# Qualcomm-AI-research/transformer-quantization

Measured on AMD Instinct MI355X. Metric: M elems/sec fake-quant fwd (BERT-base act tensor); achieved HBM GB/s vs peak, higher is better.
Workload: dtype f32; 1 GPU; BERT-base W8A8 per-tensor asym 8-bit activation fake-quant, running-minmax calibrated, fixed-range fwd, hidden [1024,512,768] bf16 per GPU (BASELINE configs[1]); storage_dtype=bf16, parallelism=dp1 (independent shards, no data-path collective)

## Files before the change

transformer-quantization_amd/csrc/tq_linear_i8.hip:

```cpp
#include <algorithm>
#include <type_traits>

#include "tq_device.h"
#include "tq_host.h"

namespace tq {

typedef int v4i __attribute__((ext_vector_type(4)));

enum { ACT_NONE = 0, ACT_RELU = 1, ACT_GELU = 2, ACT_TANH = 3 };

__device__ __forceinline__ float apply_act(float v, int act) {
  switch (act) {
    case ACT_RELU: return v > 0.0f ? v : 0.0f;
    case ACT_GELU: return 0.5f * v * (1.0f + erff(v * 0.70710678118654752440f));
    case ACT_TANH: return tanhf(v);
    default: return v;
  }
}

struct LinArgs {
  const int8_t* x;
  const int8_t* w;
  const int32_t* w_rowsum;
// ... 426 lines not shown
    if (GROUPED && p.split_out && grp == 2) w.t2sel = p.q_t2c;
    w.q1 = load_qraw(p.q_t1, 0, p.x_delta);
    w.q2 = load_qraw(w.t2sel, 0, p.x_delta);
  }
  w.st[0] = w.st[1] = w.st[2] = w.st[3] = 0.0f;
  if (!WITH_TAIL && p.stair != nullptr) {
#pragma unroll
    for (int i = 0; i < 4; ++i) w.st[i] = p.stair[i];
  }
  return w;
}

template <bool WITH_TAIL>
__device__ __forceinline__ void epilogue_arrived(EpiRaw& w) {
  w.dx = pinned_uniform(w.dx);
  w.zx = pinned_uniform(w.zx);
  qraw_arrived(w.qo);
  if (WITH_TAIL) { qraw_arrived(w.q1); qraw_arrived(w.q2); }
  else {
#pragma unroll
    for (int i = 0; i < 4; ++i) w.st[i] = pinned_uniform(w.st[i]);
  }
}

template <bool WITH_TAIL, bool SEL = false>
__device__ __forceinline__ EpiCtx epilogue_finish(const LinArgs& p, const EpiRaw& w) {
  EpiCtx c;
  c.sx = w.dx < p.x_eps ? p.x_eps : w.dx;
  const int zx = (int)clamp_nanprop(rintf(w.zx), 0.0f, grid_top(p.x_n_bits));
  c.shift = 128 - zx;
  c.qo = QP{1.f, 0.f, 0.f, 0.f};
  if (p.has_q) c.qo = qp_from_raw<SEL>(w.qsel, w.qo);
  c.qf = make_qf(c.qo);
  c.fast = p.act != ACT_TANH && (!p.has_q || c.qf.ok) && p.fast_epi != 0;
  c.stair = false;
  c.st_inv_w = c.st_c0 = c.st_nbm1 = 0.0f;
  if (!WITH_TAIL && p.stair != nullptr && p.has_q && c.fast) {
    c.st_inv_w = w.st[0]; c.st_c0 = w.st[1]; c.st_nbm1 = w.st[2];
    c.stair = w.st[3] == 1.0f && c.st_nbm1 == (float)(p.stair_bins - 1);
  }
  c.qf1 = c.qf2 = c.qf;
  if (WITH_TAIL) {
    c.qf1 = make_qf(p.on_t1 ? qp_from_raw<SEL>(p.q_t1, w.q1) : QP{1.f, 0.f, 0.f, 1.f});
    c.qf2 = make_qf(p.on_t2 ? qp_from_raw<SEL>(w.t2sel, w.q2) : QP{1.f, 0.f, 0.f, 1.f});
    c.fast = c.fast && p.act == ACT_NONE && c.qf1.ok && c.qf2.ok;
  }
  return c;
}

template <bool WITH_TAIL>
__device__ __forceinline__ EpiCtx epilogue_prepare(const LinArgs& p, uint32_t n0) {
  EpiRaw w = epilogue_fetch<WITH_TAIL>(p, n0);
  epilogue_arrived<WITH_TAIL>(w);
  return epilogue_finish<WITH_TAIL>(p, w);
}

template <int NI, int MI, int YDT, bool STAGED, bool WITH_TAIL, bool FLUSH = true, bool FPRE = false>
__device__ __forceinline__ void linear_epilogue(const LinArgs& p, v4i (&acc)[NI][MI], uint32_t n0, uint32_t m0, int r16,
                                                int kg, const EpiCtx& c, int8_t* stage = nullptr, const float* cst = nullptr,
                                                int cs = 2 * NI * 16, const f32x4 (*res_pre)[MI] = nullptr,
                                                const u32x2* stair_lds = nullptr) {
  static_assert(!(FPRE && WITH_TAIL), "class-ordered input grids: no fused tail");
  if (!c.fast) return linear_epilogue_generic<NI, MI, YDT, FPRE>(p, acc, n0, m0, r16, kg, c.qo, c.shift, c.sx, res_pre, FLUSH ? nullptr : stage);
  if (WITH_TAIL) {
#define TQ_EPI_T(Q, T) linear_epilogue_fast<NI, MI, YDT, ACT_NONE, Q, STAGED, T, FLUSH>(p, acc, n0, m0, r16, kg, c.qf, c.shift, c.sx, stage, cst, c.qf1, c.qf2, cs, res_pre)
    if (p.tail == 2) { if (p.has_q) TQ_EPI_T(true, 2); else TQ_EPI_T(false, 2); }
    else             { if (p.has_q) TQ_EPI_T(true, 1); else TQ_EPI_T(false, 1); }
#undef TQ_EPI_T
    return;
  }
#define TQ_EPI(A, Q) linear_epilogue_fast<NI, MI, YDT, A, Q, STAGED, 0, true, FPRE>(p, acc, n0, m0, r16, kg, c.qf, c.shift, c.sx, stage, cst, QF{}, QF{}, cs)
  if (STAGED && c.stair && stair_lds != nullptr) {
    linear_epilogue_stair<NI, MI, YDT, FPRE>(p, acc, n0, m0, r16, kg, c.qf, stage, cst, cs, StairRef{stair_lds, c.st_inv_w, c.st_c0, c.st_nbm1});
    return;
  }
  if (p.has_q) {
    if (p.act == ACT_GELU)      TQ_EPI(ACT_GELU, true);
    else if (p.act == ACT_RELU) TQ_EPI(ACT_RELU, true);
    else                        TQ_EPI(ACT_NONE, true);
  } else {
    if (p.act == ACT_GELU)      TQ_EPI(ACT_GELU, false);
    else if (p.act == ACT_RELU) TQ_EPI(ACT_RELU, false);
    else                        TQ_EPI(ACT_NONE, false);
  }
#undef TQ_EPI
}

template <int TN, int TM, int YDT, bool WITH_TAIL>
__global__ __launch_bounds__(kBlock) void linear_i8_k(LinArgs p) {
  constexpr int NI = TN / 16, MI = TM / 16;
  const int lane = threadIdx.x & 63;
  const uint32_t tiles_m = p.M / TM;
  const uint32_t tile = blockIdx.x * (kBlock / kWave) + (threadIdx.x >> 6);
  if (tile >= tiles_m * (p.N / TN)) return;
  const uint32_t n0 = (tile / tiles_m) * TN, m0 = (tile % tiles_m) * TM;

  const int r16 = lane & 15, kg = lane >> 4;
  const int8_t* wp = p.w + (size_t)(n0 + r16) * p.K + kg * 16;
  const int8_t* xp = p.x + (size_t)(m0 + r16) * p.K + kg * 16;

  v4i acc[NI][MI];
#pragma unroll
  for (int i = 0; i < NI; ++i)
#pragma unroll
    for (int j = 0; j < MI; ++j) acc[i][j] = v4i{0, 0, 0, 0};

  v4i fw[NI], fx[MI];
#pragma unroll
  for (int i = 0; i < NI; ++i) fw[i] = *reinterpret_cast<const v4i*>(wp + (size_t)i * 16 * p.K);
#pragma unroll
  for (int j = 0; j < MI; ++j) fx[j] = *reinterpret_cast<const v4i*>(xp + (size_t)j * 16 * p.K);

  for (uint32_t k = 64; k <= p.K; k += 64) {
    v4i nw[NI], nx[MI];
    const bool more = k < p.K;
    if (more) {
#pragma unroll
      for (int i = 0; i < NI; ++i) nw[i] = *reinterpret_cast<const v4i*>(wp + (size_t)i * 16 * p.K + k);
#pragma unroll
      for (int j = 0; j < MI; ++j) nx[j] = *reinterpret_cast<const v4i*>(xp + (size_t)j * 16 * p.K + k);
    }
#pragma unroll
    for (int i = 0; i < NI; ++i)
#pragma unroll
      for (int j = 0; j < MI; ++j)
        acc[i][j] = __builtin_amdgcn_mfma_i32_16x16x64_i8(fw[i], fx[j], acc[i][j], 0, 0, 0);
    if (more) {
#pragma unroll
      for (int i = 0; i < NI; ++i) fw[i] = nw[i];
#pragma unroll
      for (int j = 0; j < MI; ++j) fx[j] = nx[j];
    }
  }
  linear_epilogue<NI, MI, YDT, false, WITH_TAIL>(p, acc, n0, m0, r16, kg, epilogue_prepare<WITH_TAIL>(p, n0));
}

__device__ __forceinline__ void lds_dma_wait_all() { asm volatile("s_waitcnt vmcnt(0)" ::: "memory"); }

#define TQ_GLDS16(gp, lp)                                                                         \
  __builtin_amdgcn_global_load_lds((const __attribute__((address_space(1))) void*)(gp),           \
                                   (__attribute__((address_space(3))) void*)(lp), 16, 0, 0)

template <int N>
__device__ __forceinline__ void lds_dma_wait_but() {
  asm volatile("s_waitcnt vmcnt(%0)" ::"n"(N) : "memory");
}

struct ClsArgs {
  uint32_t n;
  uint32_t end_slab[TQ_CLS_MAX];
  uint32_t rep[TQ_CLS_MAX];
};

template <int WT, int YDT, bool WITH_TAIL, int NS, bool CLS, bool X16 = false>
__device__ __forceinline__ void linear_i8_lds_body(const LinArgs& p, const ClsArgs* ct, const int8_t* x_lo = nullptr) {
  static_assert(NS == 2 || NS == 8, "double buffer or the 8-stage ring");
  static_assert(!CLS || (NS == 2 && !WITH_TAIL), "class-ordered input grids: double buffer, no tail");
  static_assert(!X16 || (NS == 2 && !WITH_TAIL && !CLS), "16-bit input grids: double buffer, no tail, per-tensor");
  constexpr int BT = 2 * WT, NI = WT / 16, MI = WT / 16;
  constexpr int LPW = WT / 16;
  constexpr int OPB = BT * 128, STB = (X16 ? 3 : 2) * OPB;
  extern __shared__ __attribute__((aligned(1024))) int8_t lds_i8[];
  prefetch_kernarg<sizeof(LinArgs)>();
  const int tid = threadIdx.x, lane = tid & 63, wave = __builtin_amdgcn_readfirstlane(tid >> 6);
  const uint32_t tiles_m = p.M / BT;
  const int wn = (wave >> 1) * WT, wm = (wave & 1) * WT;
  const int r16 = lane & 15, kg = lane >> 4;
  const int swz = (r16 >> 1) & 7;
  const int off[2] = {r16 * 128 + ((kg ^ swz) << 4), r16 * 128 + (((4 + kg) ^ swz) << 4)};
  float* cst = reinterpret_cast<float*>(lds_i8 + NS * STB);
  float* csx = reinterpret_cast<float*>(lds_i8 + NS * STB + 5 * BT * 4);
  int* csh = reinterpret_cast<int*>(csx + TQ_CLS_MAX);
  int* crs = csh + TQ_CLS_MAX;
  const uint32_t cls_bytes = CLS ? 2 * TQ_CLS_MAX * 4 + ct->n * BT * 4 : 0;
  u32x2* stab = reinterpret_cast<u32x2*>(lds_i8 + NS * STB + 5 * BT * 4 + cls_bytes);
  const uint32_t nk = p.K / 128;

  {
    const uint32_t tile = blockIdx.x;
    const uint32_t n0 = (tile / tiles_m) * BT, m0 = (tile % tiles_m) * BT;
    const int8_t* wsrc[LPW];
    const int8_t* xsrc[LPW];
    const int8_t* x2src[X16 ? LPW : 1];
#pragma unroll
    for (int q = 0; q < LPW; ++q) {
      const int row = wave * (WT / 2) + q * 8 + (lane >> 3);
      const int chunk = (lane & 7) ^ ((row >> 1) & 7);
      wsrc[q] = p.w + (size_t)(n0 + row) * p.K + chunk * 16;
      xsrc[q] = p.x + (size_t)(m0 + row) * p.K + chunk * 16;
      if (X16) x2src[X16 ? q : 0] = x_lo + (size_t)(m0 + row) * p.K + chunk * 16;
    }
    auto issue = [&](int stage, uint32_t k) {
#ifdef TQ_I8_DBG_BUILD
      if (p.dbg & 2) return;
#endif
      int8_t* bw = lds_i8 + stage * STB + wave * (WT / 2) * 128;
#pragma unroll
      for (int q = 0; q < LPW; ++q) {
        TQ_GLDS16(wsrc[q] + k, bw + q * 1024);
        TQ_GLDS16(xsrc[q] + k, bw + OPB + q * 1024);
        if (X16) TQ_GLDS16(x2src[X16 ? q : 0] + k, bw + 2 * OPB + q * 1024);
      }
    };

    v4i acc[NI][MI];
    f32x4 facc[CLS ? NI : 1][CLS ? MI : 1];
    v4i acc2[X16 ? NI : 1][X16 ? MI : 1];
#pragma unroll
    for (int i = 0; i < NI; ++i)
#pragma unroll
      for (int j = 0; j < MI; ++j) acc[i][j] = v4i{0, 0, 0, 0};
    if (X16) {
#pragma unroll
      for (int i = 0; i < (X16 ? NI : 1); ++i)
#pragma unroll
        for (int j = 0; j < (X16 ? MI : 1); ++j) acc2[i][j] = v4i{0, 0, 0, 0};
    }
    if (CLS) {
#pragma unroll
      for (int i = 0; i < (CLS ? NI : 1); ++i)
#pragma unroll
        for (int j = 0; j < (CLS ? MI : 1); ++j) facc[i][j] = f32x4{-0.0f, -0.0f, -0.0f, -0.0f};
    }
    uint32_t cls = 0, cls_end = CLS ? ct->end_slab[0] : 0;

    EpiRaw eraw = epilogue_fetch<WITH_TAIL>(p, n0 + wn);
    const uint32_t ncol = n0 + (tid & (BT - 1));
    const float ld_dw = p.w_delta[p.w_n_params == 1 ? 0 : ncol], ld_b = p.bias ? p.bias[ncol] : 0.0f;
    const int ld_rs = CLS ? 0 : p.w_rowsum[ncol];
    float ld_nw = 0.0f, ld_nb = 0.0f;
    if (WITH_TAIL) { ld_nw = p.nn_w[ncol]; ld_nb = p.nn_b[ncol]; }
    if (CLS) {
      if (tid < BT)
        for (uint32_t c = 0; c < ct->n; ++c) crs[c * BT + tid] = p.w_rowsum[(size_t)c * p.N + ncol];
      if (tid == 0)
        for (uint32_t c = 0; c < ct->n; ++c) {
          const float dxc = p.x_delta[ct->rep[c]], zfc = p.x_zero_float[ct->rep[c]];
          csx[c] = dxc < p.x_eps ? p.x_eps : dxc;
          csh[c] = 128 - (int)clamp_nanprop(rintf(zfc), 0.0f, grid_top(p.x_n_bits));
        }
    }
#pragma unroll
    for (int s = 0; s < (NS == 2 ? 2 : NS - 2); ++s)
      if ((uint32_t)s < nk) issue(s, s * 128);
    epilogue_arrived<WITH_TAIL>(eraw);
    const EpiCtx ectx = epilogue_finish<WITH_TAIL, WT == 64>(p, eraw);
    if (tid < BT) {
      cst[tid] = CLS ? (ld_dw < p.w_eps ? p.w_eps : ld_dw) : ectx.sx * (ld_dw < p.w_eps ? p.w_eps : ld_dw);
      cst[BT + tid] = ld_b;
      reinterpret_cast<int*>(cst)[2 * BT + tid] = X16 ? ld_rs : ld_rs * ectx.shift;
      if (WITH_TAIL) { cst[3 * BT + tid] = ld_nw; cst[4 * BT + tid] = ld_nb; }
    }
    if (!WITH_TAIL && ectx.stair) {
      const u32x2* gtab = reinterpret_cast<const u32x2*>(p.stair + 4);
      for (uint32_t i = tid; i < p.stair_bins; i += kBlock) stab[i] = gtab[i];
    }
    for (uint32_t kb = 0; kb < nk; ++kb) {
      if (NS == 2) {
        lds_dma_wait_all();
        __syncthreads();
        if (kb > 0 && kb + 1 < nk) issue((kb + 1) & 1, (kb + 1) * 128);
      } else if ((kb & 1) == 0) {
        constexpr int IPS = 2 * LPW;
        const uint32_t rest = nk - 2 - kb;
        if (rest >= (uint32_t)(NS - 4)) lds_dma_wait_but<(NS - 4) * IPS>();
        else if (rest == 2) lds_dma_wait_but<2 * IPS>();
        else lds_dma_wait_but<0>();
        asm volatile("s_barrier" ::: "memory");
        if (kb + NS - 2 < nk) {
          issue((kb + NS - 2) % NS, (kb + NS - 2) * 128);
          issue((kb + NS - 1) % NS, (kb + NS - 1) * 128);
        }
      }
      const int8_t* bw = lds_i8 + (kb % NS) * STB + wn * 128;
      const int8_t* bx = lds_i8 + (kb % NS) * STB + OPB + wm * 128;
      v4i fw[2][NI], fx[2][MI], fx2[2][X16 ? MI : 1];
      auto load_frags = [&](int s2) {
#pragma unroll
        for (int i = 0; i < NI; ++i) fw[s2][i] = *reinterpret_cast<const v4i*>(bw + i * 2048 + off[s2]);
#pragma unroll
        for (int j = 0; j < MI; ++j) fx[s2][j] = *reinterpret_cast<const v4i*>(bx + j * 2048 + off[s2]);
        if (X16) {
#pragma unroll
          for (int j = 0; j < (X16 ? MI : 1); ++j) fx2[s2][j] = *reinterpret_cast<const v4i*>(bx + OPB + j * 2048 + off[s2]);
        }
      };
      load_frags(0);
#pragma unroll
      for (int s = 0; s < 2; ++s) {
        if (s == 0) load_frags(1);
        __builtin_amdgcn_sched_barrier(0);
#ifdef TQ_I8_DBG_BUILD
        if (p.dbg & 4) {
#pragma unroll
          for (int i = 0; i < NI; ++i) acc[i][0] = acc[i][0] + fw[s][i] + fx[s][i % MI];
          continue;
        }
#endif
#pragma unroll
        for (int i = 0; i < NI; ++i)
#pragma unroll
          for (int j = 0; j < MI; ++j)
            acc[i][j] = __builtin_amdgcn_mfma_i32_16x16x64_i8(fw[s][i], fx[s][j], acc[i][j], 0, 0, 0);
        if (X16) {
#pragma unroll
          for (int i = 0; i < (X16 ? NI : 1); ++i)
#pragma unroll
            for (int j = 0; j < (X16 ? MI : 1); ++j)
              acc2[i][j] = __builtin_amdgcn_mfma_i32_16x16x64_i8(fw[s][i], fx2[s][j], acc2[i][j], 0, 0, 0);
        }
      }
      if (CLS && kb + 1 == cls_end) {
        const float sxc = csx[cls];
        const int shc = csh[cls];
        const int* rsc = crs + cls * BT + wn;
#pragma unroll
        for (int i = 0; i < (CLS ? NI : 1); ++i) {
          const int col = i * 16 + kg * 4;
          const f32x4 sw4 = *reinterpret_cast<const f32x4*>(cst + wn + col);
          const v4i rs4 = *reinterpret_cast<const v4i*>(rsc + col);
          const f32x4 sc4 = f32x4{sxc, sxc, sxc, sxc} * sw4;
          const v4i cr4 = rs4 * v4i{shc, shc, shc, shc};
#pragma unroll
          for (int j = 0; j < (CLS ? MI : 1); ++j) {
            const v4i t = acc[i][j] + cr4;
            facc[i][j] = facc[i][j] + __builtin_convertvector(t, f32x4) * sc4;
            acc[i][j] = v4i{0, 0, 0, 0};
          }
        }
        ++cls;
        cls_end = cls < ct->n ? ct->end_slab[cls] : 0;
      }
    }
    if (CLS) {
#pragma unroll
      for (int i = 0; i < NI; ++i)
#pragma unroll
        for (int j = 0; j < MI; ++j) acc[i][j] = __builtin_bit_cast(v4i, facc[CLS ? i : 0][CLS ? j : 0]);
    }
    if (X16) {
      const double sh = (double)(ectx.shift + 32768);
#pragma unroll
      for (int i = 0; i < (X16 ? NI : 1); ++i) {
        const int col = wn + i * 16 + kg * 4;
        const f32x4 sw4 = *reinterpret_cast<const f32x4*>(cst + col);
        const v4i rs4 = *reinterpret_cast<const v4i*>(cst + 2 * BT + col);
        double cr[4];
#pragma unroll
        for (int r = 0; r < 4; ++r) cr[r] = (double)rs4[r] * sh;
#pragma unroll
        for (int j = 0; j < (X16 ? MI : 1); ++j) {
          f32x4 f;
#pragma unroll
          for (int r = 0; r < 4; ++r) {
            const double tot = __builtin_fma((double)acc[i][j][r], 256.0, (double)acc2[i][j][r]) + cr[r];
            f[r] = (float)tot * sw4[r];
          }
          acc[i][j] = __builtin_bit_cast(v4i, f);
        }
      }
    }
    __syncthreads();
#ifdef TQ_I8_DBG_BUILD
    if (p.dbg & 1) {
      if (acc[0][0][0] == 0x7fffffff) p.y_idx[0] = 1;
      return;
    }
#endif
    constexpr int kStageBytes = 32 * (WT * 4 + 16) + 32 * (WT + 16);
    static_assert(4 * kStageBytes <= 2 * STB, "output staging must fit the operand stages");
    linear_epilogue<NI, MI, YDT, true, WITH_TAIL, true, CLS || X16>(p, acc, n0 + wn, m0 + wm, r16, kg, ectx, lds_i8 + wave * kStageBytes,
                                                             cst + wn, 2 * NI * 16, nullptr, stab);
  }
}

template <int WT, int YDT, bool WITH_TAIL, int NS = 2>
__global__ __launch_bounds__(kBlock, WT == 64 ? 2 : 4) void linear_i8_lds_k(LinArgs p) {
  linear_i8_lds_body<WT, YDT, WITH_TAIL, NS, false>(p, nullptr);
}

template <int WT, int YDT>
__global__ __launch_bounds__(kBlock, WT == 64 ? 2 : 4) void linear_i8_cls_k(LinArgs p, ClsArgs ct) {
  linear_i8_lds_body<WT, YDT, false, 2, true>(p, &ct);
}

template <int WT, int YDT>
__global__ __launch_bounds__(kBlock, WT == 64 ? 2 : 3) void linear_i16x8_k(LinArgs p, const int8_t* x_lo) {
  linear_i8_lds_body<WT, YDT, false, 2, false, true>(p, nullptr, x_lo);
}

struct FfnArgs {
  const int8_t* x;
  const int8_t* w1;
  const int32_t* rs1;
  const float* b1;
  const float* w1_delta;
  uint32_t w1_n_params;
  float w1_eps;
  const float* x_delta;
  const float* x_zero_float;
  float x_eps;
  int x_n_bits;
  tq_quantizer q_mid;
  const int8_t* w2;
  const int32_t* rs2;
  LinArgs lin2;
  uint32_t M;
};

template <int NI1, int MI>
__device__ __forceinline__ void ffn_gemm1(v4i (&acc1)[NI1][MI], const int8_t* bw, const int8_t* bx, const int (&off)[2]) {
#pragma unroll
  for (int i = 0; i < NI1; ++i)
#pragma unroll
    for (int j = 0; j < MI; ++j) acc1[i][j] = v4i{0, 0, 0, 0};
#pragma unroll
  for (int s = 0; s < 2; ++s) {
    v4i fx[MI];
#pragma unroll
    for (int j = 0; j < MI; ++j) fx[j] = *reinterpret_cast<const v4i*>(bx + j * 2048 + off[s]);
#pragma unroll
    for (int i = 0; i < NI1; ++i) {
      const v4i fw = *reinterpret_cast<const v4i*>(bw + i * 2048 + off[s]);
#pragma unroll
      for (int j = 0; j < MI; ++j) acc1[i][j] = __builtin_amdgcn_mfma_i32_16x16x64_i8(fw, fx[j], acc1[i][j], 0, 0, 0);
    }
  }
}

template <int N1, int NI1, int MI, int BM>
__device__ __forceinline__ void ffn_epilogue1(const v4i (&acc1)[NI1][MI], const QP& qm, const float* c1, int8_t* hb, int col0,
                                              int chunk0, int r16, int kg) {
  const QF qf = make_qf(qm);
  const f32x2 zpb = {qm.zp, qm.zp};
  constexpr int IT = 2, NP = IT * 2 * MI;
#pragma unroll
  for (int i0 = 0; i0 < NI1; i0 += IT) {
    f32x2 v[NP], hq[NP];
#pragma unroll
    for (int ii = 0; ii < IT; ++ii) {
      const int col = col0 + (i0 + ii) * 16 + kg * 4;
      const f32x4 s4 = *reinterpret_cast<const f32x4*>(c1 + col);
      const f32x4 b4 = *reinterpret_cast<const f32x4*>(c1 + N1 + col);
      const v4i r4 = *reinterpret_cast<const v4i*>(c1 + 2 * N1 + col);
      const f32x2 sw[2] = {f32x2{s4.x, s4.y}, f32x2{s4.z, s4.w}}, bs[2] = {f32x2{b4.x, b4.y}, f32x2{b4.z, b4.w}};
#pragma unroll
      for (int j = 0; j < MI; ++j) {
        const v4i a = acc1[i0 + ii][j];
        const f32x2 lo = {(float)(a[0] + r4.x), (float)(a[1] + r4.y)};
        const f32x2 hi = {(float)(a[2] + r4.z), (float)(a[3] + r4.w)};
        v[(ii * MI + j) * 2] = lo * sw[0] + bs[0];
        v[(ii * MI + j) * 2 + 1] = hi * sw[1] + bs[1];
      }
    }
#pragma unroll
    for (int e = 0; e < NP; ++e) v[e] = f32x2{v[e].x > 0.0f ? v[e].x : 0.0f, v[e].y > 0.0f ? v[e].y : 0.0f};
    if (qf.ok) {
      qf_round2_n<NP>(v, qf, hq);
#pragma unroll
      for (int e = 0; e < NP; ++e) hq[e] = hq[e] + zpb;
    } else {
#pragma unroll
      for (int e = 0; e < NP; ++e) hq[e] = f32x2{q_index(v[e].x, qm), q_index(v[e].y, qm)};
    }
#pragma unroll
    for (int ii = 0; ii < IT; ++ii)
#pragma unroll
      for (int j = 0; j < MI; ++j) {
        const f32x2 lo = hq[(ii * MI + j) * 2], hi = hq[(ii * MI + j) * 2 + 1];
        uint32_t w = 0;
        w = __builtin_amdgcn_cvt_pk_u8_f32(lo.x, 0, w);
        w = __builtin_amdgcn_cvt_pk_u8_f32(lo.y, 1, w);
        w = __builtin_amdgcn_cvt_pk_u8_f32(hi.x, 2, w);
        w = __builtin_amdgcn_cvt_pk_u8_f32(hi.y, 3, w) ^ 0x80808080u;
        const int m = j * 16 + r16;
        *reinterpret_cast<uint32_t*>(hb + m * 128 + (((chunk0 + i0 + ii) ^ ((m >> 1) & 7)) << 4) + kg * 4) = w;
      }
  }
}

template <int NI2, int MI, int SL2, int RW, int BM>
__device__ __forceinline__ void ffn_gemm2(v4i (&acc2)[NI2][MI], const int8_t* w2, const int8_t* hbase, const int (&off)[2]) {
#pragma unroll
  for (int i = 0; i < NI2; ++i)
#pragma unroll
    for (int j = 0; j < MI; ++j) acc2[i][j] = v4i{0, 0, 0, 0};
#pragma unroll
  for (int sl = 0; sl < SL2; ++sl) {
    const int8_t* bw = w2 + sl * RW * 128;
    const int8_t* bh = hbase + sl * (BM * 128);
#pragma unroll
    for (int s = 0; s < 2; ++s) {
      v4i fw[NI2], fh[MI];
#pragma unroll
      for (int i = 0; i < NI2; ++i) fw[i] = *reinterpret_cast<const v4i*>(bw + i * 2048 + off[s]);
#pragma unroll
      for (int j = 0; j < MI; ++j) fh[j] = *reinterpret_cast<const v4i*>(bh + j * 2048 + off[s]);
#pragma unroll
      for (int i = 0; i < NI2; ++i)
#pragma unroll
        for (int j = 0; j < MI; ++j) acc2[i][j] = __builtin_amdgcn_mfma_i32_16x16x64_i8(fw[i], fh[j], acc2[i][j], 0, 0, 0);
    }
  }
}

template <int K1, int N1, int N2, int YDT, int BM>
__global__ __launch_bounds__(kBlock) void ffn_i8_k(FfnArgs p) {
  static_assert(K1 == 128 && N1 == 512 && N2 == 128, "instantiated for MobileBERT's feed-forward shape");
  static_assert(BM == 16 || BM == 32, "token rows per block");
  constexpr int MI = BM / 16;
  constexpr int NI1 = N1 / 4 / 16;
  constexpr int NI2 = N2 / 4 / 16;
  constexpr int SL2 = N1 / 128;
  constexpr int kX = 0, kH = kX + BM * 128, kW1 = kH + SL2 * BM * 128, kW1w = (N1 / 4) * 128;
  constexpr int kW2 = kW1 + 4 * kW1w, kW2w = SL2 * (N2 / 4) * 128, kC1 = kW2 + 4 * kW2w, kC2 = kC1 + 3 * N1 * 4;
  extern __shared__ __attribute__((aligned(1024))) int8_t lds_i8[];
  prefetch_kernarg<sizeof(FfnArgs)>();
  const int tid = threadIdx.x, lane = tid & 63, wave = __builtin_amdgcn_readfirstlane(tid >> 6);
  const int r16 = lane & 15, kg = lane >> 4;
  const uint32_t m0 = blockIdx.x * BM;

  {
    const int row8 = lane >> 3, slot = lane & 7;
    if (wave * 8 < BM) {
      const int row = wave * 8 + row8;
      TQ_GLDS16(p.x + (size_t)(m0 + row) * K1 + ((slot ^ ((row >> 1) & 7)) << 4), lds_i8 + kX + wave * 1024);
    }
#pragma unroll
    for (int q = 0; q < N1 / 4 / 8; ++q) {
      const int row = q * 8 + row8;
      TQ_GLDS16(p.w1 + (size_t)(wave * (N1 / 4) + row) * K1 + ((slot ^ ((row >> 1) & 7)) << 4), lds_i8 + kW1 + wave * kW1w + q * 1024);
// ... 167 lines not shown
  if (wave * 8 < BM) {
    const int row = wave * 8 + row8;
    TQ_GLDS16(st0.x + (size_t)(m0 + row) * K1 + ((slot ^ ((row >> 1) & 7)) << 4), lds_i8 + kX + wave * 1024);
  }
  issue_w1(st0);
  issue_w2(st0);
  prefetch_kernarg<4 * sizeof(FfnArgs) + sizeof(int)>();
  StageRegs g0 = fetch(st0), g1 = g0, g2 = g0, g3 = g0;
  if (nf > 1) g1 = fetch(st1);
  if (nf > 2) g2 = fetch(st2);
  if (nf > 3) g3 = fetch(st3);
  f32x4 res[NI2][MI];
#pragma unroll
  for (int i = 0; i < NI2; ++i)
    res[i][0] = *reinterpret_cast<const f32x4*>(st0.lin2.residual + (size_t)(m0 + r16) * N2 + wave * C2W + i * 16 + kg * 4);
  arrived(g0); arrived(g1); arrived(g2); arrived(g3);

  const int swz = (r16 >> 1) & 7;
  const int off[2] = {r16 * 128 + ((kg ^ swz) << 4), r16 * 128 + (((4 + kg) ^ swz) << 4)};

  auto run_stage = [&](auto fc, const FfnArgs& p, const FfnArgs& pn, const StageRegs& cur) __attribute__((always_inline)) {
    constexpr int f = decltype(fc)::value;
    const LinArgs& l2 = p.lin2;
    const bool more = f + 1 < nf;
    TQ_FSTAMP(0);
    const EpiCtx ectx = epilogue_finish<true>(l2, cur.eraw);
    const QP qm = qp_from_raw(p.q_mid, cur.mraw);
    {
      const float sx = cur.dx < p.x_eps ? p.x_eps : cur.dx;
      const int zx = (int)clamp_nanprop(rintf(cur.zf), 0.0f, grid_top(p.x_n_bits));
#pragma unroll
      for (int t = 0; t < C1W / 64; ++t) {
        const int n = wave * C1W + lane + t * 64;
        c1[n] = sx * (cur.dw1[t] < p.w1_eps ? p.w1_eps : cur.dw1[t]);
        c1[N1 + n] = cur.b1[t];
        reinterpret_cast<int*>(c1)[2 * N1 + n] = cur.rs1[t] * (128 - zx);
      }
      if (lane < C2W) {
        const int n2 = wave * C2W + lane;
        const int zm = (int)qm.zp;
        c2[n2] = qm.scale * (cur.dw2 < l2.w_eps ? l2.w_eps : cur.dw2);
        c2[N2 + n2] = cur.b2;
        reinterpret_cast<int*>(c2)[2 * N2 + n2] = cur.rs2 * (128 - zm);
        c2[3 * N2 + n2] = cur.nw;
        c2[4 * N2 + n2] = cur.nb;
      }
    }
    TQ_FSTAMP(1);
    lds_dma_wait_but<IW>();
    asm volatile("s_waitcnt lgkmcnt(0)\n\ts_barrier" ::: "memory");
    TQ_FSTAMP(2);
    v4i acc1[NI1][MI];
    ffn_gemm1<NI1, MI>(acc1, lds_i8 + kW1 + wave * kW1w, lds_i8 + kX, off);
    if (more) issue_w1(pn);
    TQ_FSTAMP(3);
    ffn_epilogue1<N1, NI1, MI, BM>(acc1, qm, c1, lds_i8 + kH + (wave * C1W / 128) * (BM * 128), wave * C1W, (wave * C1W % 128) / 16, r16, kg);
    TQ_FSTAMP(4);
    if (more) lds_dma_wait_but<IW>(); else lds_dma_wait_but<0>();
    asm volatile("s_waitcnt lgkmcnt(0)\n\ts_barrier" ::: "memory");
    TQ_FSTAMP(5);
    v4i acc2[NI2][MI];
    ffn_gemm2<NI2, MI, SL2, C2W, BM>(acc2, lds_i8 + kW2 + wave * kW2w, lds_i8 + kH, off);
    if (more) issue_w2(pn);
    TQ_FSTAMP(6);

    if (!more) {
      linear_epilogue<NI2, MI, YDT, true, true>(l2, acc2, wave * C2W, m0, r16, kg, ectx, lds_i8 + kW2 + wave * kW2w,
                                                c2 + wave * C2W, N2, res);
    } else {
      int8_t* istage = lds_i8 + kS + wave * (16 * IP);
      linear_epilogue<NI2, MI, YDT, true, true, false>(l2, acc2, wave * C2W, m0, r16, kg, ectx, istage - 16 * YP, c2 + wave * C2W, N2,
                                                       res);
      const float qs = ectx.qf2.scale.x, qz = ectx.qf2.zp;
#pragma unroll
      for (int i = 0; i < NI2; ++i) {
        const int col = i * 16 + kg * 4;
        const uint32_t w = *reinterpret_cast<const uint32_t*>(istage + r16 * IP + col);
        const uint32_t u = w ^ 0x80808080u;
        float y4[4];
#pragma unroll
        for (int r = 0; r < 4; ++r) {
          y4[r] = __builtin_fmaf(qs, (float)((u >> (8 * r)) & 0xffu) - qz, 0.0f);
          if (YDT != TQ_F32) {
            const f32x2 pr = {y4[r], 0.0f};
            const uint32_t b = __builtin_bit_cast(uint32_t, __builtin_convertvector(pr, bf16x2));
            y4[r] = __builtin_bit_cast(float, b << 16);
          }
        }
        res[i][0] = f32x4{y4[0], y4[1], y4[2], y4[3]};
        const int chunk = wave * NI2 + i;
        *reinterpret_cast<uint32_t*>(lds_i8 + kX + r16 * 128 + ((chunk ^ ((r16 >> 1) & 7)) << 4) + kg * 4) = w;
      }
    }
    TQ_FSTAMP(7);
  };
  run_stage(std::integral_constant<int, 0>{}, st0, st1, g0);
  if (nf > 1) run_stage(std::integral_constant<int, 1>{}, st1, st2, g1);
  if (nf > 2) run_stage(std::integral_constant<int, 2>{}, st2, st3, g2);
  if (nf > 3) run_stage(std::integral_constant<int, 3>{}, st3, st3, g3);
}

__global__ __launch_bounds__(kBlock) void rowsum_i8_k(const int8_t* __restrict__ w, int32_t* __restrict__ out, uint32_t N,
                                                      uint32_t K) {
  const uint32_t n = blockIdx.x * (kBlock / kWave) + (threadIdx.x >> 6);
  if (n >= N) return;
  const int lane = threadIdx.x & 63;
  int s = 0;
  for (uint32_t k = lane; k < K; k += 64) s += (int)w[(size_t)n * K + k];
#pragma unroll
  for (int o = 32; o > 0; o >>= 1) s += __shfl_xor(s, o, 64);
  if (lane == 0) out[n] = s;
}

struct TilePlan {
  bool big;
  uint32_t bt;
  uint64_t grid;
  size_t base;
};
static TilePlan tile_plan(uint64_t M, uint64_t N, uint64_t K) {
  const uint64_t tiles128 = (M / 128) * (N / 128);
  TilePlan t;
  t.big = M % 128 == 0 && N % 128 == 0 && (tiles128 >= 1024 || (K >= 512 && tiles128 >= (uint64_t)tuning("TQ_I8_BIG_MIN", 384)));
  t.bt = t.big ? 128 : 64;
  t.grid = (M / t.bt) * (N / t.bt);
  t.base = 2 * 2 * (size_t)t.bt * 128 + 5 * (size_t)t.bt * 4;
  return t;
}

template <auto Kernel>
static int reserve_lds(size_t bytes, const char* what) {
  static bool attr_set[64] = {};
  int dev = 0;
  if (hipGetDevice(&dev) != hipSuccess || dev < 0 || dev >= 64) dev = -1;
  if (dev >= 0 && attr_set[dev]) return TQ_OK;
  if (hipFuncSetAttribute(reinterpret_cast<const void*>(Kernel), hipFuncAttributeMaxDynamicSharedMemorySize, (int)bytes) != hipSuccess)
    return set_error(TQ_ELAUNCH, "%s: cannot reserve %zu bytes of LDS", what, bytes);
  if (dev >= 0) attr_set[dev] = true;
  return TQ_OK;
}

template <int YDT, bool WITH_TAIL>
static int launch_linear_t(const LinArgs& a, hipStream_t st) {
  if (a.K % 128 == 0 && a.M % 64 == 0 && a.N % 64 == 0 && tuning("TQ_I8_LDS", 1)) {
    const TilePlan t = tile_plan(a.M, a.N, a.K);
    const size_t room = (t.big ? 80 * 1024 : 40 * 1024) - 512 - t.base;
    LinArgs b = a;
    if (b.stair != nullptr && ((size_t)b.stair_bins * 8 > room || !tuning("TQ_I8_STAIR", 1))) b.stair = nullptr;
    const size_t lds = t.base + (b.stair != nullptr ? (size_t)b.stair_bins * 8 : 0) + (t.big ? (size_t)tuning("TQ_I8_LDS_PAD", 0) : 0);
    constexpr int kRing = 8;
    if (!t.big && b.stair == nullptr && a.K % 256 == 0 && a.K >= (uint32_t)tuning("TQ_I8_RING_MIN_K", 1024) &&
        t.grid <= (uint64_t)tuning("TQ_I8_RING_MAX_GRID", 256)) {
      constexpr auto k = linear_i8_lds_k<32, YDT, WITH_TAIL, kRing>;
      const size_t ring_lds = (size_t)kRing * 2 * 64 * 128 + 5 * 64 * 4;
      if (int e = reserve_lds<k>(ring_lds, "linear_i8_lds_k (ring)")) return e;
      hipLaunchKernelGGL(k, dim3((unsigned)t.grid), dim3(kBlock), ring_lds, st, b);
      return check_launch("linear_i8_lds_k (ring)");
    }
    if (!t.big && b.stair == nullptr && t.grid <= (uint64_t)tuning("TQ_I8_SMALL_MAX_GRID", 256)) {
      const uint64_t grid32 = (uint64_t)(a.M / 32) * (a.N / 32);
      const size_t lds32 = 2 * 2 * 32 * 128 + 5 * 32 * 4;
      hipLaunchKernelGGL((linear_i8_lds_k<16, YDT, WITH_TAIL>), dim3((unsigned)grid32), dim3(kBlock), lds32, st, b);
      return check_launch("linear_i8_lds_k (32 x 32 tiles)");
    }
    if (t.big) hipLaunchKernelGGL((linear_i8_lds_k<64, YDT, WITH_TAIL>), dim3((unsigned)t.grid), dim3(kBlock), lds, st, b);
    else       hipLaunchKernelGGL((linear_i8_lds_k<32, YDT, WITH_TAIL>), dim3((unsigned)t.grid), dim3(kBlock), lds, st, b);
    return check_launch("linear_i8_lds_k");
  }
  const unsigned grid = (unsigned)ceil_div((uint64_t)(a.M / 32) * (a.N / 32), kBlock / kWave);
  hipLaunchKernelGGL((linear_i8_k<32, 32, YDT, WITH_TAIL>), dim3(grid), dim3(kBlock), 0, st, a);
  return check_launch("linear_i8_k");
}

constexpr size_t kClsLds64 = 52 * 1024;
struct ClsLds {
  size_t base;
  size_t cap;
};
static ClsLds cls_lds(const TilePlan& t, uint32_t n_classes) {
  return {t.base + 2 * TQ_CLS_MAX * 4 + (size_t)n_classes * t.bt * 4, (t.big ? 80 * 1024 : kClsLds64) - 512};
}

template <int YDT>
static int launch_linear_cls(LinArgs a, const ClsArgs& ct, hipStream_t st) {
  a.fast_epi = tuning("TQ_I8_FAST_EPI", 1);
  a.dbg = 0;
  const TilePlan t = tile_plan(a.M, a.N, a.K);
  const ClsLds c = cls_lds(t, ct.n);
  if (c.base > c.cap) return set_error(TQ_EINVAL, "tq_linear_i8_cls_fwd: %u classes do not fit the LDS of a block", ct.n);
  if (a.stair != nullptr && (size_t)a.stair_bins * 8 > c.cap - c.base)
    return set_error(TQ_EINVAL, "tq_linear_i8_cls_fwd: a staircase of %u bins does not fit beside %u classes", a.stair_bins, ct.n);
  if (a.stair != nullptr && !tuning("TQ_I8_STAIR", 1)) a.stair = nullptr;
  const size_t lds = c.base + (a.stair != nullptr ? (size_t)a.stair_bins * 8 : 0);
  if (t.big) {
    hipLaunchKernelGGL((linear_i8_cls_k<64, YDT>), dim3((unsigned)t.grid), dim3(kBlock), lds, st, a, ct);
  } else {
    constexpr auto k = linear_i8_cls_k<32, YDT>;
    if (int e = reserve_lds<k>(kClsLds64, "linear_i8_cls_k")) return e;
    hipLaunchKernelGGL(k, dim3((unsigned)t.grid), dim3(kBlock), lds, st, a, ct);
  }
  return check_launch("linear_i8_cls_k");
}

constexpr size_t kX16Bt = 64;
static ClsLds x16_lds() { return {2 * 3 * kX16Bt * 128 + 5 * kX16Bt * 4, 80 * 1024 - 512}; }

template <int YDT>
static int launch_linear_x16(LinArgs a, const int8_t* x_lo, hipStream_t st) {
  a.fast_epi = tuning("TQ_I8_FAST_EPI", 1);
  a.dbg = 0;
  const ClsLds c = x16_lds();
  const uint64_t grid = (a.M / kX16Bt) * (a.N / kX16Bt);
  if (a.stair != nullptr && (size_t)a.stair_bins * 8 > c.cap - c.base)
    return set_error(TQ_EINVAL, "tq_linear_i16x8_fwd: a staircase of %u bins does not fit the LDS of a block", a.stair_bins);
  if (a.stair != nullptr && !tuning("TQ_I8_STAIR", 1)) a.stair = nullptr;
  const size_t lds = c.base + (a.stair != nullptr ? (size_t)a.stair_bins * 8 : 0);
  constexpr auto k = linear_i16x8_k<32, YDT>;
  if (int e = reserve_lds<k>(c.cap, "linear_i16x8_k")) return e;
  hipLaunchKernelGGL(k, dim3((unsigned)grid), dim3(kBlock), lds, st, a, x_lo);
  return check_launch("linear_i16x8_k");
}

static int launch_linear(LinArgs a, int y_dtype, tq_stream_t stream) {
  a.fast_epi = tuning("TQ_I8_FAST_EPI", 1);
  a.dbg = tuning("TQ_I8_DBG", 0);
  hipStream_t st = static_cast<hipStream_t>(stream);
  if (y_dtype == TQ_F32) return a.tail ? launch_linear_t<TQ_F32, true>(a, st) : launch_linear_t<TQ_F32, false>(a, st);
  return a.tail ? launch_linear_t<TQ_BF16, true>(a, st) : launch_linear_t<TQ_BF16, false>(a, st);
}

struct LinShape {
  uint32_t mn, k;
  const char* rule;
};
constexpr LinShape kAnyShape{32, 64, "M,N % 32, K % 64"};
constexpr LinShape kTiledShape{64, 128, "M, N % 64, K % 128"};
constexpr LinShape kGroupedShape{64, 128, "M % 64, K % 128"};

static int lin_args(LinArgs& a, const char* who, const LinShape& s, const int8_t* x, const int8_t* w, const int32_t* w_rowsum,
                    const float* bias, void* y, int8_t* y_idx, bool need_y, int y_dtype, uint64_t M, uint64_t N, uint64_t K,
                    const float* x_delta, const float* x_zero_float, int x_n_bits, float x_eps, const float* w_delta,
                    uint64_t w_n_params, float w_eps, int act, int max_x_bits = 8) {
  TQ_REQUIRE(x && w && w_rowsum && (need_y ? y != nullptr : y || y_idx) && x_delta && x_zero_float && w_delta, "%s: NULL pointer", who);
  TQ_REQUIRE(y_dtype == TQ_F32 || y_dtype == TQ_BF16, "%s: y dtype must be fp32 or bf16", who);
  TQ_REQUIRE(M % s.mn == 0 && N % s.mn == 0 && K % s.k == 0 && K >= s.k && K <= 16384 && M < (1u << 31) && N < (1u << 31),
             "%s: unsupported shape M=%llu N=%llu K=%llu (%s)", who, (unsigned long long)M, (unsigned long long)N,
             (unsigned long long)K, s.rule);
  TQ_REQUIRE(x_n_bits >= 1 && x_n_bits <= max_x_bits, "%s: input quantizer must have <= %d bits", who, max_x_bits);
  TQ_REQUIRE(w_n_params == 1 || w_n_params == N, "%s: weight scales must be per-tensor or per-output-channel", who);
  TQ_REQUIRE(act >= ACT_NONE && act <= ACT_TANH, "%s: unknown activation %d", who, act);
  TQ_REQUIRE(aligned16(x) && aligned16(w) && (y == nullptr || aligned16(y)), "%s: 16-byte alignment required", who);
  a.x = x; a.w = w; a.w_rowsum = w_rowsum; a.bias = bias; a.y = y; a.y_idx = y_idx;
  a.M = (uint32_t)M; a.N = (uint32_t)N; a.K = (uint32_t)K;
  a.x_delta = x_delta; a.x_zero_float = x_zero_float; a.x_eps = x_eps; a.x_n_bits = x_n_bits;
  a.w_delta = w_delta; a.w_n_params = (uint32_t)w_n_params; a.w_eps = w_eps; a.act = act;
  a.group_cols = (uint32_t)N;
  return TQ_OK;
}

static int check_y_idx(const char* who, const int8_t* y_idx, const tq_quantizer* q, bool groups = false) {
  if (y_idx == nullptr || (q != nullptr && !q->symmetric && q->n_bits <= 8)) return TQ_OK;
  return set_error(TQ_EINVAL, groups ? "%s: y_idx needs asymmetric <= 8-bit output quantizers"
                                     : "%s: y_idx needs an asymmetric <= 8-bit output quantizer", who);
}

static int quantizer_slot(const char* who, const char* what, const tq_quantizer* q, uint64_t n, tq_quantizer& slot, int& on) {
  on = q != nullptr;
  if (q == nullptr) return TQ_OK;
  if (int e = check_quantizer(q, n, who)) return e;
  TQ_REQUIRE(q->n_params == 1, "%s: per-tensor %s only", who, what);
  slot = *q;
  return TQ_OK;
}

static int nonorm_quantizers(LinArgs& a, const char* who, uint64_t n, const tq_quantizer* q_dense, const tq_quantizer* q_sum,
                             const tq_quantizer* q_out) {
  if (int e = quantizer_slot(who, "quantizers", q_dense, n, a.q_out, a.has_q)) return e;
  if (int e = quantizer_slot(who, "quantizers", q_sum, n, a.q_t1, a.on_t1)) return e;
  return quantizer_slot(who, "quantizers", q_out, n, a.q_t2, a.on_t2);
}

static int lin_out(LinArgs& a, const char* who, const tq_quantizer* q_out, const void* act_stair, uint32_t stair_bins) {
  TQ_REQUIRE(act_stair == nullptr || (q_out != nullptr && stair_bins >= 64 && stair_bins <= 2048 && aligned16(act_stair)),
             "%s: the staircase needs an output quantizer, 64..2048 bins and 16-byte alignment", who);
  if (int e = check_y_idx(who, a.y_idx, q_out)) return e;
  if (int e = quantizer_slot(who, "output quantizer", q_out, (uint64_t)a.M * a.N, a.q_out, a.has_q)) return e;
  a.stair = static_cast<const float*>(act_stair);
  a.stair_bins = stair_bins;
  return TQ_OK;
}

}

using namespace tq;

extern "C" int tq_rowsum_i8(const int8_t* w_idx, int32_t* rowsum, uint64_t N, uint64_t K, tq_stream_t stream) {
  TQ_REQUIRE(w_idx && rowsum && N >= 1 && K >= 1, "tq_rowsum_i8: bad argument");
  hipLaunchKernelGGL(rowsum_i8_k, dim3((unsigned)ceil_div(N, kBlock / kWave)), dim3(kBlock), 0,
                     static_cast<hipStream_t>(stream), w_idx, rowsum, (uint32_t)N, (uint32_t)K);
  return check_launch("rowsum_i8_k");
}

extern "C" int tq_linear_i8_grouped_fwd(const int8_t* x_idx, const int8_t* w_idx, const int32_t* w_rowsum,
                                        const float* bias, void* y, int8_t* y_idx, int y_dtype, uint64_t M, uint64_t N,
                                        uint64_t K, const float* x_delta, const float* x_zero_float, int x_n_bits,
                                        float x_eps, const float* w_delta, float w_eps, int activation,
                                        uint64_t n_groups, const tq_quantizer* const* q_out, tq_stream_t stream) {
// ... 286 lines not shown
```

Baseline: 1.567 million M elems/s.

## Add eight-wave variant of the int8 ring GEMM kernel and make it default

New measurement: 1.530 million M elems/s. 0.976x the previous value.

```diff
diff --git a/transformer-quantization_amd/csrc/tq_linear_i8.hip b/transformer-quantization_amd/csrc/tq_linear_i8.hip
--- a/transformer-quantization_amd/csrc/tq_linear_i8.hip
+++ b/transformer-quantization_amd/csrc/tq_linear_i8.hip
@@ -602,19 +602,21 @@
   uint32_t rep[TQ_CLS_MAX];
 };
 
-template <int WT, int YDT, bool WITH_TAIL, int NS, bool CLS, bool X16 = false>
+template <int WT, int YDT, bool WITH_TAIL, int NS, bool CLS, bool X16 = false, int RW = 4>
 __device__ __forceinline__ void linear_i8_lds_body(const LinArgs& p, const ClsArgs* ct, const int8_t* x_lo = nullptr) {
   static_assert(NS == 2 || NS == 8, "double buffer or the 8-stage ring");
+  static_assert(RW == 4 || (RW == 8 && NS == 8 && WT == 32), "eight waves: the ring of 64 x 64 tiles only");
   static_assert(!CLS || (NS == 2 && !WITH_TAIL), "class-ordered input grids: double buffer, no tail");
   static_assert(!X16 || (NS == 2 && !WITH_TAIL && !CLS), "16-bit input grids: double buffer, no tail, per-tensor");
-  constexpr int BT = 2 * WT, NI = WT / 16, MI = WT / 16;
-  constexpr int LPW = WT / 16;
+  constexpr int BT = 2 * WT, NI = WT / 16, MI = RW == 8 ? WT / 32 : WT / 16;
+  constexpr int RPW = BT / RW;
+  constexpr int LPW = RPW / 8;
   constexpr int OPB = BT * 128, STB = (X16 ? 3 : 2) * OPB;
   extern __shared__ __attribute__((aligned(1024))) int8_t lds_i8[];
   prefetch_kernarg<sizeof(LinArgs)>();
   const int tid = threadIdx.x, lane = tid & 63, wave = __builtin_amdgcn_readfirstlane(tid >> 6);
   const uint32_t tiles_m = p.M / BT;
-  const int wn = (wave >> 1) * WT, wm = (wave & 1) * WT;
+  const int wn = RW == 8 ? (wave >> 2) * WT : (wave >> 1) * WT, wm = RW == 8 ? (wave & 3) * (WT / 2) : (wave & 1) * WT;
   const int r16 = lane & 15, kg = lane >> 4;
   const int swz = (r16 >> 1) & 7;
   const int off[2] = {r16 * 128 + ((kg ^ swz) << 4), r16 * 128 + (((4 + kg) ^ swz) << 4)};
@@ -634,7 +636,7 @@
     const int8_t* x2src[X16 ? LPW : 1];
 #pragma unroll
     for (int q = 0; q < LPW; ++q) {
-      const int row = wave * (WT / 2) + q * 8 + (lane >> 3);
+      const int row = wave * RPW + q * 8 + (lane >> 3);
       const int chunk = (lane & 7) ^ ((row >> 1) & 7);
       wsrc[q] = p.w + (size_t)(n0 + row) * p.K + chunk * 16;
       xsrc[q] = p.x + (size_t)(m0 + row) * p.K + chunk * 16;
@@ -644,7 +646,7 @@
 #ifdef TQ_I8_DBG_BUILD
       if (p.dbg & 2) return;
 #endif
-      int8_t* bw = lds_i8 + stage * STB + wave * (WT / 2) * 128;
+      int8_t* bw = lds_i8 + stage * STB + wave * RPW * 128;
 #pragma unroll
       for (int q = 0; q < LPW; ++q) {
         TQ_GLDS16(wsrc[q] + k, bw + q * 1024);
@@ -703,7 +705,7 @@
     }
     if (!WITH_TAIL && ectx.stair) {
       const u32x2* gtab = reinterpret_cast<const u32x2*>(p.stair + 4);
-      for (uint32_t i = tid; i < p.stair_bins; i += kBlock) stab[i] = gtab[i];
+      for (uint32_t i = tid; i < p.stair_bins; i += RW * 64) stab[i] = gtab[i];
     }
     for (uint32_t kb = 0; kb < nk; ++kb) {
       if (NS == 2) {
@@ -817,8 +819,9 @@
       return;
     }
 #endif
-    constexpr int kStageBytes = 32 * (WT * 4 + 16) + 32 * (WT + 16);
-    static_assert(4 * kStageBytes <= 2 * STB, "output staging must fit the operand stages");
+    constexpr int kStageRows = RW == 8 ? 16 : 32;
+    constexpr int kStageBytes = kStageRows * (WT * 4 + 16) + kStageRows * (WT + 16);
+    static_assert(RW * kStageBytes <= 2 * STB, "output staging must fit the operand stages");
     linear_epilogue<NI, MI, YDT, true, WITH_TAIL, true, CLS || X16>(p, acc, n0 + wn, m0 + wm, r16, kg, ectx, lds_i8 + wave * kStageBytes,
                                                              cst + wn, 2 * NI * 16, nullptr, stab);
   }
@@ -827,6 +830,11 @@
 template <int WT, int YDT, bool WITH_TAIL, int NS = 2>
 __global__ __launch_bounds__(kBlock, WT == 64 ? 2 : 4) void linear_i8_lds_k(LinArgs p) {
   linear_i8_lds_body<WT, YDT, WITH_TAIL, NS, false>(p, nullptr);
+}
+
+template <int YDT, bool WITH_TAIL>
+__global__ __launch_bounds__(2 * kBlock, 2) void linear_i8_ring8w_k(LinArgs p) {
+  linear_i8_lds_body<32, YDT, WITH_TAIL, 8, false, false, 8>(p, nullptr);
 }
 
 template <int WT, int YDT>
@@ -1300,7 +1308,13 @@
     if (!t.big && b.stair == nullptr && a.K % 256 == 0 && a.K >= (uint32_t)tuning("TQ_I8_RING_MIN_K", 1024) &&
         t.grid <= (uint64_t)tuning("TQ_I8_RING_MAX_GRID", 256)) {
       constexpr auto k = linear_i8_lds_k<32, YDT, WITH_TAIL, kRing>;
+      constexpr auto k8 = linear_i8_ring8w_k<YDT, WITH_TAIL>;
       const size_t ring_lds = (size_t)kRing * 2 * 64 * 128 + 5 * 64 * 4;
+      if (tuning("TQ_I8_RING_WAVES", 8) != 4) {
+        if (int e = reserve_lds<k8>(ring_lds, "linear_i8_ring8w_k")) return e;
+        hipLaunchKernelGGL(k8, dim3((unsigned)t.grid), dim3(2 * kBlock), ring_lds, st, b);
+        return check_launch("linear_i8_ring8w_k");
+      }
       if (int e = reserve_lds<k>(ring_lds, "linear_i8_lds_k (ring)")) return e;
       hipLaunchKernelGGL(k, dim3((unsigned)t.grid), dim3(kBlock), ring_lds, st, b);
       return check_launch("linear_i8_lds_k (ring)");
```
